# TheRealShamsaba/KnightVision

Hardware: AMD Instinct MI355X
Metric: MCTS simulations/sec + self-play games/hour (higher is better)
Workload: dtype fp32

## Files before the change

### include/kv.h

```cpp
#ifndef KV_H
#define KV_H

#include <stddef.h>
#include <stdint.h>

#ifdef __cplusplus
extern "C" {
#endif

#define KV_OK 0
#define KV_EINVAL -1
#define KV_ENOMEM -2
#define KV_EHIP -3
#define KV_EOVERFLOW -4

const char* kv_last_error(void);
int kv_version(void);

typedef struct kv_net kv_net;

size_t kv_net_packed_size(void);
int kv_net_create(int device, kv_net** out);
int kv_net_load(kv_net* net, const float* packed, size_t n_floats);
int kv_net_forward(kv_net* net, const float* planes_dev, int B, float* policy_dev, float* value_dev, void* stream);
// ... 152 lines not shown
} kv_search_result;
int kv_search(kv_engine* e, const int8_t* states , int n,
              const kv_search_params* p, kv_search_result* out );
size_t kv_sizeof_search_result(void);

int kv_search_advance(kv_engine* e, int n, const int32_t* edge , int8_t* states_out );
int kv_search_continue(kv_engine* e, int n, const kv_search_params* p, kv_search_result* out ,
                       int32_t* kept );
int kv_search_tree_size(kv_engine* e, int i, int32_t* nodes, int32_t* edges);


int kv_dev_valid_moves(int device, const int8_t* states, int n, uint16_t* moves_out, int cap, int* n_moves,
                       int8_t* states_after, uint8_t* in_check);
int kv_dev_attacks(int device, const int8_t* states, int n, uint64_t* attacked);
int kv_dev_make_move(int device, int8_t* states, const int* index, int n);
int kv_dev_dirichlet(int device, const uint64_t* seeds, int n, double alpha, int k, int draws, double* out,
                     int64_t* attempts, double* tail);
int kv_host_libm(int op, const double* x, const double* y, int n, double* out);
int kv_dev_py_random(int device, const uint64_t* seeds, int n, int count, double* out);
int kv_dev_wino88i(int device, const double* V, int rows, const double* U, int K, int digits, int seg, double* M,
                   int8_t* v_digits, int* v_exp);
int kv_dev_wino88i32_out(int device, const float* M, int rows, const float* scale, const float* shift,
                         const float* resid, int fused, float* Y, int8_t* v_digits, int* v_exp);
int kv_dev_wino88r_out(int device, const double* M, int rows, const float* scale, const float* shift,
                       const float* resid, int fused, float* Y, int8_t* v_digits, int* v_exp);
int kv_dev_i8gemm_bench(int device, int rows, int K, int variant, int iters, float* avg_us, float* M_out);
int kv_dev_gemm_clock(int device, int rows, int digits, double seconds, double* out);
int kv_dev_out_phases(int device, int rows, int resid, int r3, unsigned long long* stamps, float* us);

#define KV_PGN_OUTCOME_NONE (-128)
typedef struct kv_pgn_record {
    char fen[100];
    char san[12];
    int32_t outcome;
    int32_t game;
} kv_pgn_record;
int kv_pgn_extract(const char* text, size_t len, kv_pgn_record* out, size_t cap, size_t* n_out, size_t* consumed,
                   int64_t* n_games);
int kv_fen_codes(const char* fens, size_t stride, int n, int8_t* codes);
int kv_san_move_index(const char* fens, size_t fen_stride, const char* sans, size_t san_stride, int n,
                      int32_t* out);
int kv_chess_perft(const char* fen, int depth, uint64_t* nodes);
int kv_chess_san(const char* fen, const char* san_in, char* san_out, size_t san_cap, char* fen_after, size_t fen_cap);
int kv_chess_fen(const char* fen_in, char* fen_out, size_t cap);

int kv_tr_conv3x3_f16(const void* x_dev, int n, int ci, const void* w_dev, const float* bias_dev, int co,
// ... 38 lines not shown
```

### knightvision_amd/_lib.py

```python
from __future__ import annotations

import ctypes as C
import os

HERE = os.path.dirname(os.path.abspath(__file__))
LIB_PATH = os.environ.get("KV_LIB_PATH") or os.path.join(HERE, "libkv.so")

_lib = None


class KVError(RuntimeError):
    pass


class Config(C.Structure):
    _fields_ = [("device", C.c_int), ("slots", C.c_int), ("n_games", C.c_int64), ("game_id_base", C.c_int64),
                ("game_id_stride", C.c_int64), ("seed", C.c_uint64), ("seed_mode", C.c_int),
                ("max_moves", C.c_int), ("batch", C.c_int), ("eps", C.c_double), ("alpha", C.c_double),
                ("sims", C.c_int), ("c_puct", C.c_float), ("eval_mode", C.c_int), ("record_cap", C.c_int64),
                ("recycle", C.c_int), ("precision", C.c_int), ("algo", C.c_int), ("tree_edge_cap", C.c_int),
                ("keep_root_visits", C.c_int), ("reuse_tree", C.c_int)]


class Record(C.Structure):
# ... 97 lines not shown
        "kv_root_moves": ([vp, P(C.c_uint16), sz, P(sz)], i),
        "kv_root_moves_device": ([vp, vp, sz, P(sz), vp], i),
        "kv_records_device": ([vp, vp, sz, P(sz), vp], i),
        "kv_sync": ([vp], i),
        "kv_reset_records": ([vp], i),
        "kv_destroy": ([vp], None),
        "kv_search": ([vp, P(C.c_int8), i, P(SearchParams), P(SearchResult)], i),
        "kv_sizeof_search_result": ([], sz),
        "kv_search_advance": ([vp, i, P(C.c_int32), P(C.c_int8)], i),
        "kv_search_continue": ([vp, i, P(SearchParams), P(SearchResult), P(C.c_int32)], i),
        "kv_search_tree_size": ([vp, i, P(C.c_int32), P(C.c_int32)], i),
        "kv_dev_valid_moves": ([i, P(C.c_int8), i, P(C.c_uint16), i, P(i), P(C.c_int8), P(C.c_uint8)], i),
        "kv_dev_make_move": ([i, P(C.c_int8), P(i), i], i),
        "kv_dev_attacks": ([i, P(C.c_int8), i, P(C.c_uint64)], i),
        "kv_dev_dirichlet": ([i, P(C.c_uint64), i, C.c_double, i, i, P(C.c_double), P(i64), P(C.c_double)], i),
        "kv_dev_py_random": ([i, P(C.c_uint64), i, i, P(C.c_double)], i),
        "kv_host_libm": ([i, P(C.c_double), P(C.c_double), i, P(C.c_double)], i),
        "kv_dev_wino88i": ([i, P(C.c_double), i, P(C.c_double), i, i, i, P(C.c_double), P(C.c_int8), P(i)], i),
        "kv_dev_i8gemm_bench": ([i, i, i, i, i, P(C.c_float), P(C.c_float)], i),
        "kv_dev_gemm_clock": ([i, i, i, C.c_double, P(C.c_double)], i),
        "kv_dev_out_phases": ([i, i, i, i, P(C.c_uint64), P(C.c_float)], i),
        "kv_dev_wino88i32_out": ([i, P(C.c_float), i, P(C.c_float), P(C.c_float), P(C.c_float), i, P(C.c_float),
                                  P(C.c_int8), P(i)], i),
        "kv_dev_wino88r_out": ([i, P(C.c_double), i, P(C.c_float), P(C.c_float), P(C.c_float), i, P(C.c_float),
                                P(C.c_int8), P(i)], i),
        "kv_pgn_extract": ([C.c_char_p, sz, P(PgnRecord), sz, P(sz), P(sz), P(i64)], i),
        "kv_fen_codes": ([C.c_char_p, sz, i, P(C.c_int8)], i),
        "kv_san_move_index": ([C.c_char_p, sz, C.c_char_p, sz, i, P(C.c_int32)], i),
        "kv_chess_perft": ([C.c_char_p, i, P(C.c_uint64)], i),
        "kv_chess_san": ([C.c_char_p, C.c_char_p, C.c_char_p, sz, C.c_char_p, sz], i),
        "kv_chess_fen": ([C.c_char_p, C.c_char_p, sz], i),
        "kv_tr_conv3x3_f16": ([vp, i, i, vp, vp, i, vp, vp], i),
        "kv_tr_conv3x3_add_f16": ([vp, i, i, vp, vp, i, vp, vp, vp], i),
        "kv_tr_conv_weights_f16": ([vp, i, i, i, vp, vp, vp], i),
        "kv_tr_wgrad_workspace": ([i, i, i, P(i)], sz),
        "kv_tr_conv3x3_wgrad_f16": ([vp, vp, i, i, i, i, vp, vp, sz, vp], i),
        "kv_tr_bn_workspace": ([i, i], sz),
        "kv_tr_bn_stats_f16": ([vp, i, i, C.c_float, vp, vp, vp, vp, sz, vp], i),
        "kv_tr_bn_apply_f16": ([vp, i, i, vp, vp, vp, vp, vp, i, vp, vp], i),
        "kv_tr_bn_backward_f16": ([vp, vp, vp, i, i, i, vp, vp, vp, vp, vp, vp, vp, vp, vp, sz, vp], i),
        "kv_tr_channel_sum_f16": ([vp, i, i, vp, vp, sz, vp], i),
        "kv_tr_planes_to_nhwc": ([vp, i, i, vp, vp], i),
        "kv_tr_head1x1_f16": ([vp, i, vp, vp, vp, vp], i),
        "kv_tr_head1x1_workspace": ([i], sz),
        "kv_tr_head1x1_backward_f16": ([vp, vp, i, vp, vp, vp, vp, vp, sz, vp], i),
        "kv_tr_policy_loss_f16": ([vp, vp, vp, vp, vp, i, vp, vp, vp, vp], i),
        "kv_tr_policy_loss_backward_f16": ([vp, vp, vp, vp, vp, i, vp, vp, vp, vp, vp, vp], i),
    }
    for name, (args, res) in sig.items():
        if not hasattr(L, name):
            continue
        f = getattr(L, name)
        f.argtypes = args
        f.restype = res
    return L


EXPORTED = ["kv_last_error", "kv_version", "kv_net_packed_size", "kv_net_create", "kv_net_load", "kv_net_forward",
            "kv_net_forward_boards", "kv_net_forward_boards_legal", "kv_net_set_timing", "kv_net_last_timing", "kv_net_destroy", "kv_net_set_precision", "kv_net_set_algo",
            "kv_net_calibration", "kv_engine_calibration",
            "kv_create",
            "kv_load_weights", "kv_run", "kv_set_max_moves", "kv_records", "kv_games", "kv_stats_get", "kv_sizeof_config", "kv_sizeof_stats", "kv_root_visits", "kv_root_visits_device", "kv_root_moves", "kv_root_moves_device", "kv_records_device", "kv_sync", "kv_reset_records", "kv_destroy",
            "kv_search", "kv_sizeof_search_result", "kv_search_advance", "kv_search_continue", "kv_search_tree_size",
            "kv_dev_valid_moves", "kv_dev_make_move", "kv_dev_attacks", "kv_dev_dirichlet", "kv_dev_py_random", "kv_host_libm",
            "kv_dev_wino88i", "kv_dev_wino88i32_out", "kv_dev_wino88r_out", "kv_dev_i8gemm_bench",
            "kv_dev_gemm_clock", "kv_dev_out_phases",
            "kv_pgn_extract", "kv_fen_codes", "kv_san_move_index", "kv_chess_perft", "kv_chess_san", "kv_chess_fen",
            "kv_tr_conv3x3_f16", "kv_tr_conv3x3_add_f16", "kv_tr_conv_weights_f16", "kv_tr_wgrad_workspace", "kv_tr_conv3x3_wgrad_f16",
            "kv_tr_bn_workspace", "kv_tr_bn_stats_f16", "kv_tr_bn_apply_f16", "kv_tr_bn_backward_f16",
            "kv_tr_channel_sum_f16", "kv_tr_planes_to_nhwc", "kv_tr_head1x1_f16", "kv_tr_head1x1_workspace",
            "kv_tr_head1x1_backward_f16", "kv_tr_policy_loss_f16", "kv_tr_policy_loss_backward_f16"]


def lib():
    global _lib
    if _lib is None:
        import torch
        if not os.path.exists(LIB_PATH):
            raise KVError(f"{LIB_PATH} is missing: run `python -c 'import __graft_entry__ as g; g.build()'` "
                          "(the HIP library is required; there is no CPU fallback)")
        L = _declare(C.CDLL(LIB_PATH))
        if hasattr(L, "kv_sizeof_search_result"):
            assert L.kv_sizeof_search_result() == C.sizeof(SearchResult), "kv_search_result: ctypes mirror differs"
        if hasattr(L, "kv_sizeof_config"):
            assert L.kv_sizeof_config() == C.sizeof(Config), "kv_config: ctypes mirror differs"
            assert L.kv_sizeof_stats() == C.sizeof(Stats), "kv_stats: ctypes mirror differs"
        _lib = L
    return _lib
# ... 7 lines not shown
```

### knightvision_amd/csrc/kv_nn.hip

```cpp
#include <hip/hip_runtime.h>
#include <math.h>
#include <stdarg.h>
#include <stdlib.h>
#include <string.h>

#include <algorithm>
#include <chrono>
#include <mutex>
#include <set>
#include <utility>
#include <vector>

#include "kv_common.h"
#include "kv_wino.h"
#include "kv_wino88.h"
#include "kv_wino88d.h"
#include "kv_wino88i.h"
#include "kv_ref64.h"

namespace kv {

static thread_local char g_err[512];

void set_error(const char* fmt, ...) {
// ... 215 lines not shown
                                                           float* out) {
    const size_t i = (size_t)blockIdx.x * blockDim.x + threadIdx.x;
    if (i >= n4) return;
    const f32x4* sl = (const f32x4*)slab + i;
    f32x4 v = sl[0];
    for (int s0 = 1; s0 < splits; s0 += kReduceBatch) {
        f32x4 p[kReduceBatch];
#pragma unroll
        for (int k = 0; k < kReduceBatch; ++k)
            if (s0 + k < splits) p[k] = sl[(size_t)(s0 + k) * n4];
#pragma unroll
        for (int k = 0; k < kReduceBatch; ++k)
            if (s0 + k < splits) v += p[k];
    }
    const int c = (int)((i * 4) % (size_t)cout);
    const f32x4 sc = *(const f32x4*)(scale + c), sh = *(const f32x4*)(shift + c);
    f32x4 o = v * sc + sh;
    if (resid) o += ((const f32x4*)resid)[i];
#pragma unroll
    for (int e = 0; e < 4; ++e) o[e] = o[e] > 0.f ? o[e] : 0.f;
    ((f32x4*)out)[i] = o;
}

__global__ __launch_bounds__(1024) void heads_kernel(const float* __restrict__ X, const float* __restrict__ hw,
                                                     const float* __restrict__ hs, const float* __restrict__ hb,
                                                     const float* __restrict__ v1wT, const float* __restrict__ v1b,
                                                     const float* __restrict__ v2w, const float* __restrict__ v2b,
                                                     float* __restrict__ pfeat, float* __restrict__ value) {
    __shared__ float s_pf[128];
    __shared__ float s_v[64];
    __shared__ float s_h[512];
    __shared__ float s_red[8];
    const int b = blockIdx.x, t = threadIdx.x;
    const int p = t >> 4, q = t & 15;
    const float* xp = X + ((size_t)b * 64 + p) * 512;
    float a0 = 0.f, a1 = 0.f, a2 = 0.f;
#pragma unroll
    for (int j = 0; j < 8; ++j) {
        const int c = q * 4 + 64 * j;
        const f32x4 x = *(const f32x4*)(xp + c);
        const f32x4 w0 = *(const f32x4*)(hw + c);
        const f32x4 w1 = *(const f32x4*)(hw + 512 + c);
        const f32x4 w2 = *(const f32x4*)(hw + 1024 + c);
#pragma unroll
        for (int e = 0; e < 4; ++e) {
            a0 += x[e] * w0[e];
            a1 += x[e] * w1[e];
            a2 += x[e] * w2[e];
        }
    }
#pragma unroll
    for (int m = 1; m < 16; m <<= 1) {
        a0 += __shfl_xor(a0, m);
        a1 += __shfl_xor(a1, m);
        a2 += __shfl_xor(a2, m);
    }
    if (q == 0) {
        const float p0 = a0 * hs[0] + hb[0], p1 = a1 * hs[1] + hb[1], v = a2 * hs[2] + hb[2];
        s_pf[p] = p0 > 0.f ? p0 : 0.f;
        s_pf[64 + p] = p1 > 0.f ? p1 : 0.f;
        s_v[p] = v > 0.f ? v : 0.f;
    }
    __syncthreads();
    if (t < 128) pfeat[(size_t)b * 128 + t] = s_pf[t];
    if (t < 512) {
        float hsum = v1b[t];
#pragma unroll 16
        for (int k = 0; k < 64; ++k) hsum += v1wT[k * 512 + t] * s_v[k];
        s_h[t] = hsum > 0.f ? hsum : 0.f;
    }
    __syncthreads();
    if (t < 256) {
        float part = v2w[t] * s_h[t] + v2w[t + 256] * s_h[t + 256];
#pragma unroll
        for (int m = 32; m >= 1; m >>= 1) part += __shfl_xor(part, m);
        if ((t & 63) == 0) s_red[t >> 6] = part;
    }
    __syncthreads();
    if (t == 0) value[b] = tanhf(s_red[0] + s_red[1] + s_red[2] + s_red[3] + v2b[0]);
}

__global__ __launch_bounds__(256) void policy_fc_kernel(const float* __restrict__ pfeat,
                                                        const float* __restrict__ w, const float* __restrict__ bias,
                                                        float* __restrict__ logits, int nb) {
    const int lane = threadIdx.x & 63, wave = threadIdx.x >> 6;
    const int h = lane >> 5, li = lane & 31;
    const int n0 = blockIdx.x * 128 + wave * 32;
    const int b0 = blockIdx.y * 32;
    const int arow = min(b0 + li, nb - 1);
    const float* ap = pfeat + (size_t)arow * 128 + 4 * h;
    const float* bp = w + (size_t)(n0 + li) * 128 + 4 * h;
    f32x16 acc;
#pragma unroll
    for (int r = 0; r < 16; ++r) acc[r] = 0.f;
    f32x4 a[16], v[16];
#pragma unroll
    for (int s = 0; s < 16; ++s) {
        a[s] = *(const f32x4*)(ap + 8 * s);
        v[s] = *(const f32x4*)(bp + 8 * s);
    }
#pragma unroll
    for (int s = 0; s < 16; ++s)
// ... 343 lines not shown
static int net_reserve(kv_net* net, int nb_pad) {
    KV_REQUIRE(nb_pad <= kMaxBoards, KV_EINVAL, "kv_net: %d boards per forward (at most %d)", nb_pad, kMaxBoards);
    if (nb_pad <= net->cap) return KV_OK;
    int cap = nb_pad < 64 ? 64 : nb_pad;
    (void)hipFree(net->x16); (void)hipFree(net->X); (void)hipFree(net->T); (void)hipFree(net->pfeat);
    (void)hipFree(net->ev8); (void)hipFree(net->evmax8);
    net->x16 = net->X = net->T = net->pfeat = nullptr;
    net->ev8 = nullptr;
    net->evmax8 = nullptr;
    net->cap = 0;
    KV_HIP(hipMalloc(&net->x16, (size_t)cap * 64 * 16 * 4));
    KV_HIP(hipMalloc(&net->X, (size_t)cap * 64 * 512 * 4));
    KV_HIP(hipMalloc(&net->T, (size_t)cap * 64 * 512 * 4));
    KV_HIP(hipMalloc(&net->pfeat, (size_t)cap * 128 * 4));
    KV_HIP(hipMalloc(&net->ev8, (size_t)cap * kv::W88_XI * 2 * sizeof(int)));
    KV_HIP(hipMalloc(&net->evmax8, (size_t)cap * kv::W88_XI * sizeof(unsigned)));
    if (!net->slab)
        KV_HIP(hipMalloc(&net->slab, (size_t)(144 / kSplitKt) * kSplitMaxBoards * 64 * 512 * 4));
    net->cap = cap;
    return KV_OK;
}

static int net_heads(kv_net* net, int nb, float* policy, float* value, hipStream_t st);

template <int K, int WR, int WC, int MT, int NT, int CK, int LDS_PAD, int XI>
static int launch_wino_gemm_t(const float* V, const float* U, float* M, int rows, int stride, hipStream_t st,
                              int xi0 = 0, int nxi = XI) {
    using T = kv::WinoTile<WR, WC, MT, NT, CK>;
    constexpr size_t bytes = T::BYTES + LDS_PAD;
    KV_HIP(lds_opt_in((const void*)kv::wino_gemm_kernel<K, WR, WC, MT, NT, CK, XI>, (int)bytes));
    const int nwg = nxi * (rows / T::WM) * (512 / T::WN);
    KV_REQUIRE(rows % T::WM == 0 && nwg % 8 == 0 && xi0 >= 0 && nxi > 0 && xi0 + nxi <= XI, KV_EINVAL,
               "wino gemm: rows %d vs tile %d, points [%d, %d)", rows, T::WM, xi0, xi0 + nxi);
    hipLaunchKernelGGL((kv::wino_gemm_kernel<K, WR, WC, MT, NT, CK, XI>), dim3(nwg), dim3(T::THREADS), bytes, st, V,
                       U, M, rows, 512, stride, xi0);
    KV_HIP(hipGetLastError());
    return KV_OK;
}

static bool debug_skip_transforms() {
    static const int v = [] {
        const char* e = getenv("KV_DEBUG_SKIP_TRANSFORMS");
        return e && e[0] == '1' ? 1 : 0;
    }();
    return v != 0;
}
// ... 534 lines not shown
                                                                      kv::W88_XI, net->V8, net->ev8, st)))
            return rc;
    } else if (slice && v64) {
        KV_REQUIRE(K == 256, KV_EINVAL, "wino88i32v: the output kernels write the digits of K 512");
        if ((rc = launch_wino88i_slice<256, D>((const double*)net->V256, rows, stride, kv::W88_XI, net->V8, net->ev8,
                                               st)))
            return rc;
    } else if (slice) {
        const float* Vsrc = K == 256 ? (const float*)net->V256 : (const float*)net->V;
        rc = K == 256 ? launch_wino88i_slice<256, D>(Vsrc, rows, stride, kv::W88_XI, net->V8, net->ev8, st)
             : seg    ? launch_wino88i_slice<512, D, float, 2>(Vsrc, rows, stride, kv::W88_XI, net->V8, net->ev8, st)
                      : launch_wino88i_slice<512, D>(Vsrc, rows, stride, kv::W88_XI, net->V8, net->ev8, st);
        if (rc) return rc;
    }
    const int8_t* U = (r3 ? net->U88r3 : net->U88i32) + net->uoff88[l] * D;
    const int* eu = (r3 ? net->eu88r3 : net->eu88i32) + net->euoff[l];
    rc = K == 256 ? i8f32_gemm<256>(net->V8, net->ev8, U, eu, M, rows, stride, false, st, r3)
                  : i8f32_gemm<512>(net->V8, net->ev8, U, eu, M, rows, stride, seg, st, r3);
    if (rc) return rc;
    if (mark && net->res_b) KV_HIP(hipEventRecord(net->res_b, st));
    return KV_OK;
}

static int wino88i32_blocks(kv_net* net, int nb, bool mark, bool v64, hipStream_t st, bool r3 = false) {
    const int rows = nb, stride = rows;
    float* V = (float*)net->V;
    const float* M = (const float*)net->Mw;
    const bool sf = i8f32_form().slice && !v64 && !r3, seg = i8f32_form().seg && !v64 && !r3;
    int8_t* V8 = net->V8;
    int* ev = net->ev8;
    int rc;
    if ((rc = wino88i32_gemm_layer(net, 1, 256, rows, stride, true, false, v64, st, r3))) return rc;
    rc = v64  ? launch_wino88i32v_out<false, true>(net, 1, M, nb, stride, nullptr, net->X, V8, ev, st)
         : sf ? launch_wino88_out<false, true, true>(net, 1, M, nb, stride, nullptr, net->X, V, st)
              : launch_wino88i32_out<false, true>(net, 1, M, nb, stride, nullptr, net->X, V8, ev, seg, st, r3);
    if (rc) return rc;
    if (mark && net->timing) KV_HIP(hipEventRecord(net->ev[1], st));
    for (int r = 0; r < 5; ++r) {
        const int l1 = 2 + 2 * r, l2 = 3 + 2 * r;
        const bool m = mark && r == 2;
        if ((rc = wino88i32_gemm_layer(net, l1, 512, rows, stride, sf, m, v64, st, r3))) return rc;
        rc = v64  ? launch_wino88i32v_out<false, false>(net, l1, M, nb, stride, nullptr, nullptr, V8, ev, st)
             : sf ? launch_wino88_out<false, false, true>(net, l1, M, nb, stride, nullptr, nullptr, V, st)
                  : launch_wino88i32_out<false, false>(net, l1, M, nb, stride, nullptr, nullptr, V8, ev, seg, st, r3);
        if (rc) return rc;
        if ((rc = wino88i32_gemm_layer(net, l2, 512, rows, stride, sf, false, v64, st, r3))) return rc;
        if (r == 4)
            rc = launch_wino88_out<true, true, false>(net, l2, M, nb, stride, net->X, net->X, nullptr, st);
        else
            rc = v64  ? launch_wino88i32v_out<true, true>(net, l2, M, nb, stride, net->X, net->X, V8, ev, st)
                 : sf ? launch_wino88_out<true, true, true>(net, l2, M, nb, stride, net->X, net->X, V, st)
                      : launch_wino88i32_out<true, true>(net, l2, M, nb, stride, net->X, net->X, V8, ev, seg, st, r3);
        if (rc) return rc;
    }
    if (mark && net->timing) KV_HIP(hipEventRecord(net->ev[2], st));
    return KV_OK;
}

struct WsNeed {
    size_t b[4];
};
static WsNeed ws_need(int path) {
    constexpr size_t f = 4, d = 8, P88 = kv::W88_XI;
    switch (path) {
        case KV_PATH_WINO88: return {{P88 * 512 * f, P88 * 512 * f, P88 * 256 * f, 0}};
        case KV_PATH_WINO88_F64: return {{P88 * 512 * d, P88 * 512 * d, P88 * 256 * d, 0}};
        case KV_PATH_WINO88_I8: return {{0, P88 * 512 * d, P88 * 256 * d, P88 * 512 * kv::kI8Digits}};
        case KV_PATH_WINO88_I8R: return {{0, P88 * 512 * d, P88 * 256 * d, P88 * 512 * 4}};
        case KV_PATH_WINO88_I8F32:
            return {{i8f32_form().slice ? P88 * 512 * f : 0, P88 * 512 * f, P88 * 256 * f,
                     P88 * 512 * kv::kI8DigitsF32}};
        case KV_PATH_WINO88_I8F32V: return {{0, P88 * 512 * f, P88 * 256 * d, P88 * 512 * kv::kI8DigitsF32}};
        case KV_PATH_WINO88_I8F32R3: return {{0, P88 * 512 * f, P88 * 256 * f, P88 * 512 * kv::kI8DigitsF32}};
        default: return {{0, 0, 0, 0}};
    }
}

static int net_reserve_ws(kv_net* net, int path) {
    void** buf[4] = {&net->V, &net->Mw, &net->V256, (void**)&net->V8};
    const WsNeed n = ws_need(path);
    for (int i = 0; i < 4; ++i) {
        const size_t need = n.b[i] * (size_t)net->cap;
        if (need <= net->ws_cap[i]) continue;
        (void)hipFree(*buf[i]);
        *buf[i] = nullptr;
        net->ws_cap[i] = 0;
        KV_HIP(hipMalloc(buf[i], need));
        net->ws_cap[i] = need;
    }
    return KV_OK;
}

static int net_tower_wino(kv_net* net, int nb_pad, int path, bool v256_ready, hipStream_t st) {
    int rc;
    net->dom_path = path;
    net->dom_launches = 1;
    t_dom_kernel = nullptr;
    if (path == KV_PATH_WINO88 || path == KV_PATH_WINO88_F64 || path == KV_PATH_WINO88_I8 ||
        path == KV_PATH_WINO88_I8R || path == KV_PATH_WINO88_I8F32 || path == KV_PATH_WINO88_I8F32V ||
        path == KV_PATH_WINO88_I8F32R3) {
        const bool f64 = path == KV_PATH_WINO88_F64 || path == KV_PATH_WINO88_I8 || path == KV_PATH_WINO88_I8R ||
                         path == KV_PATH_WINO88_I8F32V;
        if (!v256_ready) {
            if (f64)
                hipLaunchKernelGGL(kv::wino88d_in_kernel<256>, dim3(1, nb_pad), dim3(256), 0, st, net->T, nb_pad,
                                   (double*)net->V256);
            else
                hipLaunchKernelGGL(kv::wino88_in_kernel<256>, dim3(1, nb_pad), dim3(256), 0, st, net->T, nb_pad,
                                   (float*)net->V256);
            KV_HIP(hipGetLastError());
        }
        if ((rc = path == KV_PATH_WINO88_I8F32    ? wino88i32_blocks(net, nb_pad, true, false, st)
                  : path == KV_PATH_WINO88_I8F32R3 ? wino88i32_blocks(net, nb_pad, true, false, st, true)
                  : path == KV_PATH_WINO88_I8F32V ? wino88i32_blocks(net, nb_pad, true, true, st)
                  : path == KV_PATH_WINO88_I8  ? wino88i_blocks(net, nb_pad, true, false, st)
                  : path == KV_PATH_WINO88_I8R ? wino88i_blocks(net, nb_pad, true, true, st)
                  : path == KV_PATH_WINO88_F64 ? wino88d_blocks(net, nb_pad, true, st)
                                               : wino88_blocks(net, nb_pad, true, st)))
            return rc;
        net->dom_flop = 2.0 * kv::W88_XI * nb_pad * 512.0 * 512.0;
        net->dom_kernel = t_dom_kernel ? t_dom_kernel : "?";
        net->dom_algo = KV_ALGO_WINOGRAD88;
        net->dom_split = path != KV_PATH_WINO88 ? 0 : (nb_pad % 128 == 0 ? wino88_split_points(nb_pad) : kv::W88_XI);
        return KV_OK;
    }
    KV_REQUIRE(false, KV_EINVAL, "kv_net: conv path %d is not a Winograd tower", path);
}

static int net_tower(kv_net* net, int nb, int nb_pad, const int8_t* boards, float* policy, float* value,
                     hipStream_t st) {
    const float* W = net->w;
    const kv::PackOffsets& o = net->off;
    int rc;
    const bool tm = net->timing;
    const int path = path_for(net, nb);
    KV_REQUIRE(net->built[path], KV_EINVAL, "kv_net: conv path %d has no weights (load the net after choosing it)",
               path);
    KV_REQUIRE(nb_pad <= net->cap, KV_EINVAL, "kv_net: %d boards over the reserved %d", nb_pad, net->cap);
    if ((rc = net_reserve_ws(net, path))) return rc;
    if (tm) KV_HIP(hipEventRecord(net->ev[0], st));
    bool v256_ready = false;
    if (boards) {
        if (path == KV_PATH_WINO88 || path == KV_PATH_WINO88_I8F32 || path == KV_PATH_WINO88_I8F32R3)
            hipLaunchKernelGGL(kv::stem_kernel<4>, dim3(4, nb_pad / 2), dim3(256), 0, st, boards, nb, net->stemT,
                               W + o.scale[0], W + o.shift[0], (float*)net->V256, nb_pad, nullptr);
        else if (path == KV_PATH_WINO88_F64 || path == KV_PATH_WINO88_I8 || path == KV_PATH_WINO88_I8R ||
                 path == KV_PATH_WINO88_I8F32V)
            hipLaunchKernelGGL(kv::stem_kernel<5>, dim3(4, nb_pad / 2), dim3(256), 0, st, boards, nb, net->stemT,
                               W + o.scale[0], W + o.shift[0], (float*)net->V256, nb_pad, nullptr);
        else
            hipLaunchKernelGGL(kv::stem_kernel<0>, dim3(4, nb_pad / 2), dim3(256), 0, st, boards, nb, net->stemT,
                               W + o.scale[0], W + o.shift[0], net->T, nb_pad * 4, nullptr);
        KV_HIP(hipGetLastError());
        v256_ready = path != KV_PATH_DIRECT;
    } else if ((rc = launch_conv<16, 16, false>(net->x16, W + o.w[0], W + o.scale[0], W + o.shift[0], nullptr,
                                                net->T, 256, nb_pad, nullptr, st))) {
        return rc;
    }
    if (path_is_wino(path)) {
        if ((rc = net_tower_wino(net, nb_pad, path, v256_ready, st))) return rc;
        return net_heads(net, nb, policy, value, st);
    }
    if ((rc = launch_conv<256, 32, false>(net->T, W + o.w[1], W + o.scale[1], W + o.shift[1], nullptr, net->X, 512,
                                          nb_pad, net->slab, st)))
        return rc;
    if (tm) KV_HIP(hipEventRecord(net->ev[1], st));
    if (net->res_a) KV_HIP(hipEventRecord(net->res_a, st));
    for (int r = 0; r < 5; ++r) {
        const int l1 = 2 + 2 * r, l2 = 3 + 2 * r;
        if ((rc = launch_conv<512, 32, false>(net->X, W + o.w[l1], W + o.scale[l1], W + o.shift[l1], nullptr, net->T,
                                              512, nb_pad, net->slab, st)))
            return rc;
        if ((rc = launch_conv<512, 32, true>(net->T, W + o.w[l2], W + o.scale[l2], W + o.shift[l2], net->X, net->X,
                                             512, nb_pad, net->slab, st)))
            return rc;
    }
    if (tm) KV_HIP(hipEventRecord(net->ev[2], st));
    if (net->res_b) KV_HIP(hipEventRecord(net->res_b, st));
    net->dom_algo = KV_ALGO_DIRECT;
    net->dom_path = KV_PATH_DIRECT;
    net->dom_split = 0;
    net->dom_kernel = "conv3x3_kernel<512,32>";
    net->dom_launches = 10;
    net->dom_flop = (double)nb_pad * 64 * 512 * 4608 * 2;
    return net_heads(net, nb, policy, value, st);
}

static int net_heads(kv_net* net, int nb, float* policy, float* value, hipStream_t st) {
    const float* W = net->w;
    const kv::PackOffsets& o = net->off;
    hipLaunchKernelGGL(kv::heads_kernel, dim3(nb), dim3(1024), 0, st, net->X, W + o.head_w, W + o.head_scale,
                       W + o.head_shift, net->v1wT, W + o.vfc1_b, W + o.vfc2_w, W + o.vfc2_b, net->pfeat, value);
    KV_HIP(hipGetLastError());
    if (net->legal.out) {
        hipLaunchKernelGGL(kv::policy_legal_kernel, dim3(nb), dim3(64), 0, st, net->pfeat, W + o.pfc_w, W + o.pfc_b,
                           net->legal.moves, net->legal.n, net->legal.maxm, net->legal.out);
    } else {
        hipLaunchKernelGGL(kv::policy_fc_kernel, dim3(4096 / 128, (nb + 31) / 32), dim3(256), 0, st, net->pfeat,
                           W + o.pfc_w, W + o.pfc_b, policy, nb);
    }
    KV_HIP(hipGetLastError());
    return KV_OK;
}

static size_t wino_offsets(size_t* uoff, int nxi) {
    size_t tot = 0;
    for (int l = 1; l < 12; ++l) {
        uoff[l] = tot;
        tot += (size_t)nxi * kv::kConv[l].cout * kv::kConv[l].cin;
    }
    return tot;
}

static int ensure_path(kv_net* net, int path) {
    if (net->built[path]) return KV_OK;
    if (path == KV_PATH_WINO88_I8F32V) {
// ... 611 lines not shown
        }
        KV_HIP(hipGetLastError());
    } else {
        if (resid)
            hipLaunchKernelGGL((kv::wino88_out_kernel<true, true, true>), dim3(512 / 256, rows), dim3(256), 0, 0,
                               dm.p, rows, sc, sh, dy.p, dy.p, dv.p);
        else
            hipLaunchKernelGGL((kv::wino88_out_kernel<false, true, true>), dim3(512 / 256, rows), dim3(256), 0, 0,
                               dm.p, rows, sc, sh, nullptr, dy.p, dv.p);
        KV_HIP(hipGetLastError());
        int rc = seg  ? launch_wino88i_slice<512, kv::kI8DigitsF32, float, 2>(dv.p, rows, rows, kv::W88_XI, v8.p, ev.p, 0)
                 : r3 ? launch_wino88i_slice<512, kv::kI8DigitsF32, float, 1, false, true>(dv.p, rows, rows, kv::W88_XI,
                                                                                           v8.p, ev.p, 0)
                      : launch_wino88i_slice<512, kv::kI8DigitsF32>(dv.p, rows, rows, kv::W88_XI, v8.p, ev.p, 0);
        if (rc) return rc;
    }
    KV_HIP(hipDeviceSynchronize());
    KV_HIP(hipMemcpy(Y, dy.p, ny * sizeof(float), hipMemcpyDeviceToHost));
    KV_HIP(hipMemcpy(v_digits, v8.p, nm * kv::kI8DigitsF32, hipMemcpyDeviceToHost));
    KV_HIP(hipMemcpy(v_exp, ev.p, (size_t)kv::W88_XI * rows * (seg ? 2 : 1) * sizeof(int), hipMemcpyDeviceToHost));
    return KV_OK;
}

int kv_dev_wino88r_out(int device, const double* M, int rows, const float* scale, const float* shift,
                       const float* resid, int fused, float* Y, int8_t* v_digits, int* v_exp) {
    KV_REQUIRE(M && scale && shift && Y && v_digits && v_exp && rows > 0 && rows % 128 == 0 && rows <= kMaxBoards,
               KV_EINVAL, "kv_dev_wino88r_out: bad arguments (rows %d: a multiple of 128, at most %d)", rows,
               kMaxBoards);
    KV_HIP(hipSetDevice(device));
    const size_t nm = (size_t)kv::W88_XI * rows * 512, ny = (size_t)rows * 64 * 512;
    kv::DevBuf<double> dm, dv;
    kv::DevBuf<float> dsc, dsh, dy;
    kv::DevBuf<int8_t> v8;
    kv::DevBuf<int> ev;
    KV_HIP(dm.alloc(nm));
    KV_HIP(dsc.alloc(512));
    KV_HIP(dsh.alloc(512));
    KV_HIP(dy.alloc(ny));
    KV_HIP(v8.alloc(nm * 4));
    KV_HIP(ev.alloc((size_t)kv::W88_XI * rows));
    KV_HIP(hipMemcpy(dm.p, M, nm * sizeof(double), hipMemcpyHostToDevice));
    KV_HIP(hipMemcpy(dsc.p, scale, 512 * sizeof(float), hipMemcpyHostToDevice));
    KV_HIP(hipMemcpy(dsh.p, shift, 512 * sizeof(float), hipMemcpyHostToDevice));
    if (resid)
        KV_HIP(hipMemcpy(dy.p, resid, ny * sizeof(float), hipMemcpyHostToDevice));
    else
// ... 356 lines not shown
```

### knightvision_amd/csrc/kv_wino88i.h

```cpp
#pragma once
#include <hip/hip_runtime.h>

#include "kv_common.h"
#include "kv_wino88.h"
#include "kv_wino88d.h"

namespace kv {

constexpr int kI8Digits = 5;
constexpr int kI8DigitsF32 = 4;

typedef int i8x16_t __attribute__((ext_vector_type(4)));
typedef int i32x16_t __attribute__((ext_vector_type(16)));

__device__ inline int i8_row_exponent(unsigned m) {
    if (!m) return 0;
    return (int)(m >> 20) - 1022 + ((m & 0xFE000u) == 0xFE000u ? 1 : 0);
}

__device__ inline int i8_row_exponent_f32(unsigned m) {
    if (!m) return 0;
    return (int)(m >> 23) - 126 + ((m & 0x7F0000u) == 0x7F0000u ? 1 : 0);
}

// ... 1716 lines not shown
            const int xi = a * 10 + bb;
            const unsigned P = i8f32_digits<R3>(vk[aa][bb], exs[xi]);
            {
                const unsigned T4 = i8_quad_transpose(P, lane);
                if constexpr (!R3)
                    __builtin_nontemporal_store(T4, &dst[(off0 + (unsigned)xi * xstride) >> 2]);
                else if (q < 3)
                    dst[(off0 + (unsigned)xi * xstride) >> 2] = T4;
            }
        }
    }
    if constexpr (STAMP) {
        st[4] = __builtin_amdgcn_s_memtime();
        asm volatile("s_waitcnt vmcnt(0)" ::: "memory");
        st[5] = __builtin_amdgcn_s_memtime();
        if (stamper) {
            unsigned long long* o = kOutStamps[b][w == 0 ? 0 : 1];
#pragma unroll
            for (int k = 0; k < 6; ++k) o[k] = st[k];
        }
    }
}

template <bool RESID, bool WRITE_Y, bool R3 = false>
__global__ __launch_bounds__(1024) void wino88i32_outp_kernel(const float* __restrict__ M, int rows,
                                                              const float* __restrict__ scale,
                                                              const float* __restrict__ shift, const float* resid,
                                                              float* Y, int8_t* __restrict__ V8,
                                                              int* __restrict__ ex) {
#pragma clang fp contract(off)
    constexpr int NK = 512 / 32, NW = 16, NSLOT = 3, SLOT = 20 * 2048;
    extern __shared__ __attribute__((aligned(16))) char lds_outp[];
    unsigned(*red)[2][5][16] = (unsigned(*)[2][5][16])(lds_outp + NSLOT * SLOT);
    int* exs = (int*)(lds_outp + NSLOT * SLOT + NW * 2 * 5 * 16 * 4);
    const int lane = threadIdx.x & 63, w = threadIdx.x >> 6, h = lane >> 5;
    const int wu = __builtin_amdgcn_readfirstlane(w);
    const int c = w * 32 + (lane & 31);
    const int G = (int)gridDim.x;
    const int nbw = ((int)rows - (int)blockIdx.x + G - 1) / G;
    const int nsteps = 5 * nbw;
    const int npieces = wu < 8 ? 3 : 2;
    const float sc = scale[c], sh = shift[c];
    const unsigned xs = (unsigned)rows * 512;
    auto issue = [&](int t) {
        if (t >= nsteps) return;
        const int b = (int)blockIdx.x + (t / 5) * G, jj = t % 5;
// ... 251 lines not shown
```

Before: 318,500.

## Fuse stem with int8 Winograd input and last output transform with heads

Adds a stem_r3 kernel that computes the stem convolution and writes int8 Winograd digits directly, skipping the fp32 V256 buffer and the separate slicing pass for large batches on the R3 path. Adds a fused kernel that runs the final residual Winograd output transform and the policy/value heads per board in LDS, so the last activation is not written to global memory and re-read. The heads math is switched to explicit FMAs, which may change numerics slightly. Test entry points for both fused paths are exported.

```diff
diff --git a/include/kv.h b/include/kv.h
--- a/include/kv.h
+++ b/include/kv.h
@@ -198,6 +198,10 @@
                    int8_t* v_digits, int* v_exp);
 int kv_dev_wino88i32_out(int device, const float* M, int rows, const float* scale, const float* shift,
                          const float* resid, int fused, float* Y, int8_t* v_digits, int* v_exp);
+int kv_dev_tower_front(int device, const int8_t* boards, int nb, int rows, const float* wT, const float* scale,
+                       const float* shift, int fused, int8_t* v_digits, int* v_exp);
+int kv_dev_tower_back(int device, const float* M, int rows, const float* scale, const float* shift,
+                      const float* resid, const float* heads, int fused, float* pfeat, float* value);
 int kv_dev_wino88r_out(int device, const double* M, int rows, const float* scale, const float* shift,
                        const float* resid, int fused, float* Y, int8_t* v_digits, int* v_exp);
 int kv_dev_i8gemm_bench(int device, int rows, int K, int variant, int iters, float* avg_us, float* M_out);
diff --git a/knightvision_amd/_lib.py b/knightvision_amd/_lib.py
--- a/knightvision_amd/_lib.py
+++ b/knightvision_amd/_lib.py
@@ -143,6 +143,10 @@
         "kv_dev_out_phases": ([i, i, i, i, P(C.c_uint64), P(C.c_float)], i),
         "kv_dev_wino88i32_out": ([i, P(C.c_float), i, P(C.c_float), P(C.c_float), P(C.c_float), i, P(C.c_float),
                                   P(C.c_int8), P(i)], i),
+        "kv_dev_tower_front": ([i, P(C.c_int8), i, i, P(C.c_float), P(C.c_float), P(C.c_float), i, P(C.c_int8),
+                                P(i)], i),
+        "kv_dev_tower_back": ([i, P(C.c_float), i, P(C.c_float), P(C.c_float), P(C.c_float), P(C.c_float), i,
+                               P(C.c_float), P(C.c_float)], i),
         "kv_dev_wino88r_out": ([i, P(C.c_double), i, P(C.c_float), P(C.c_float), P(C.c_float), i, P(C.c_float),
                                 P(C.c_int8), P(i)], i),
         "kv_pgn_extract": ([C.c_char_p, sz, P(PgnRecord), sz, P(sz), P(sz), P(i64)], i),
@@ -184,7 +188,7 @@
             "kv_load_weights", "kv_run", "kv_set_max_moves", "kv_records", "kv_games", "kv_stats_get", "kv_sizeof_config", "kv_sizeof_stats", "kv_root_visits", "kv_root_visits_device", "kv_root_moves", "kv_root_moves_device", "kv_records_device", "kv_sync", "kv_reset_records", "kv_destroy",
             "kv_search", "kv_sizeof_search_result", "kv_search_advance", "kv_search_continue", "kv_search_tree_size",
             "kv_dev_valid_moves", "kv_dev_make_move", "kv_dev_attacks", "kv_dev_dirichlet", "kv_dev_py_random", "kv_host_libm",
-            "kv_dev_wino88i", "kv_dev_wino88i32_out", "kv_dev_wino88r_out", "kv_dev_i8gemm_bench",
+            "kv_dev_wino88i", "kv_dev_wino88i32_out", "kv_dev_wino88r_out", "kv_dev_tower_front", "kv_dev_tower_back", "kv_dev_i8gemm_bench",
             "kv_dev_gemm_clock", "kv_dev_out_phases",
             "kv_pgn_extract", "kv_fen_codes", "kv_san_move_index", "kv_chess_perft", "kv_chess_san", "kv_chess_fen",
             "kv_tr_conv3x3_f16", "kv_tr_conv3x3_add_f16", "kv_tr_conv_weights_f16", "kv_tr_wgrad_workspace", "kv_tr_conv3x3_wgrad_f16",
diff --git a/knightvision_amd/csrc/kv_nn.hip b/knightvision_amd/csrc/kv_nn.hip
--- a/knightvision_amd/csrc/kv_nn.hip
+++ b/knightvision_amd/csrc/kv_nn.hip
@@ -261,18 +261,19 @@
     ((f32x4*)out)[i] = o;
 }
 
-__global__ __launch_bounds__(1024) void heads_kernel(const float* __restrict__ X, const float* __restrict__ hw,
-                                                     const float* __restrict__ hs, const float* __restrict__ hb,
-                                                     const float* __restrict__ v1wT, const float* __restrict__ v1b,
-                                                     const float* __restrict__ v2w, const float* __restrict__ v2b,
-                                                     float* __restrict__ pfeat, float* __restrict__ value) {
+__device__ inline void heads_board(const float* xb, int b, const float* __restrict__ hw,
+                                   const float* __restrict__ hs, const float* __restrict__ hb,
+                                   const float* __restrict__ v1wT, const float* __restrict__ v1b,
+                                   const float* __restrict__ v2w, const float* __restrict__ v2b,
+                                   float* __restrict__ pfeat, float* __restrict__ value) {
+#pragma clang fp contract(off)
     __shared__ float s_pf[128];
     __shared__ float s_v[64];
     __shared__ float s_h[512];
     __shared__ float s_red[8];
-    const int b = blockIdx.x, t = threadIdx.x;
+    const int t = threadIdx.x;
     const int p = t >> 4, q = t & 15;
-    const float* xp = X + ((size_t)b * 64 + p) * 512;
+    const float* xp = xb + (size_t)p * 512;
     float a0 = 0.f, a1 = 0.f, a2 = 0.f;
 #pragma unroll
     for (int j = 0; j < 8; ++j) {
@@ -283,9 +284,9 @@
         const f32x4 w2 = *(const f32x4*)(hw + 1024 + c);
 #pragma unroll
         for (int e = 0; e < 4; ++e) {
-            a0 += x[e] * w0[e];
-            a1 += x[e] * w1[e];
-            a2 += x[e] * w2[e];
+            a0 = __builtin_fmaf(x[e], w0[e], a0);
+            a1 = __builtin_fmaf(x[e], w1[e], a1);
+            a2 = __builtin_fmaf(x[e], w2[e], a2);
         }
     }
 #pragma unroll
@@ -295,7 +296,8 @@
         a2 += __shfl_xor(a2, m);
     }
     if (q == 0) {
-        const float p0 = a0 * hs[0] + hb[0], p1 = a1 * hs[1] + hb[1], v = a2 * hs[2] + hb[2];
+        const float p0 = __builtin_fmaf(a0, hs[0], hb[0]), p1 = __builtin_fmaf(a1, hs[1], hb[1]),
+                    v = __builtin_fmaf(a2, hs[2], hb[2]);
         s_pf[p] = p0 > 0.f ? p0 : 0.f;
         s_pf[64 + p] = p1 > 0.f ? p1 : 0.f;
         s_v[p] = v > 0.f ? v : 0.f;
@@ -305,18 +307,50 @@
     if (t < 512) {
         float hsum = v1b[t];
 #pragma unroll 16
-        for (int k = 0; k < 64; ++k) hsum += v1wT[k * 512 + t] * s_v[k];
+        for (int k = 0; k < 64; ++k) hsum = __builtin_fmaf(v1wT[k * 512 + t], s_v[k], hsum);
         s_h[t] = hsum > 0.f ? hsum : 0.f;
     }
     __syncthreads();
     if (t < 256) {
-        float part = v2w[t] * s_h[t] + v2w[t + 256] * s_h[t + 256];
+        float part = __builtin_fmaf(v2w[t], s_h[t], v2w[t + 256] * s_h[t + 256]);
 #pragma unroll
         for (int m = 32; m >= 1; m >>= 1) part += __shfl_xor(part, m);
         if ((t & 63) == 0) s_red[t >> 6] = part;
     }
     __syncthreads();
     if (t == 0) value[b] = tanhf(s_red[0] + s_red[1] + s_red[2] + s_red[3] + v2b[0]);
+}
+
+__global__ __launch_bounds__(1024) void heads_kernel(const float* __restrict__ X, const float* __restrict__ hw,
+                                                     const float* __restrict__ hs, const float* __restrict__ hb,
+                                                     const float* __restrict__ v1wT, const float* __restrict__ v1b,
+                                                     const float* __restrict__ v2w, const float* __restrict__ v2b,
+                                                     float* __restrict__ pfeat, float* __restrict__ value) {
+    const int b = blockIdx.x;
+    heads_board(X + (size_t)b * 64 * 512, b, hw, hs, hb, v1wT, v1b, v2w, v2b, pfeat, value);
+}
+
+constexpr int kOutHeadsLds = 64 * 512 * 4;
+template <bool YNT>
+__global__ __launch_bounds__(1024) void wino88_out_heads_kernel(
+    const float* __restrict__ M, int rows, const float* __restrict__ scale, const float* __restrict__ shift,
+    const float* __restrict__ resid, const float* __restrict__ hw, const float* __restrict__ hs,
+    const float* __restrict__ hb, const float* __restrict__ v1wT, const float* __restrict__ v1b,
+    const float* __restrict__ v2w, const float* __restrict__ v2b, float* __restrict__ pfeat,
+    float* __restrict__ value) {
+    extern __shared__ __attribute__((aligned(16))) float xs[];
+    const int lane = threadIdx.x & 63, w = threadIdx.x >> 6, h = lane >> 5;
+    const int c = w * 32 + (lane & 31), b = blockIdx.x;
+    {
+        float x2[4][8];
+        wino88_out_plane_half<true, false, false, 0, YNT>(M, rows, b, c, h, scale[c], shift[c], resid, nullptr, x2);
+#pragma unroll
+        for (int ii = 0; ii < 4; ++ii)
+#pragma unroll
+            for (int j = 0; j < 8; ++j) xs[((4 * h + ii) * 8 + j) * 512 + c] = x2[ii][j];
+    }
+    __syncthreads();
+    heads_board(xs, b, hw, hs, hb, v1wT, v1b, v2w, v2b, pfeat, value);
 }
 
 __global__ __launch_bounds__(256) void policy_fc_kernel(const float* __restrict__ pfeat,
@@ -706,6 +740,7 @@
 }
 
 static int net_heads(kv_net* net, int nb, float* policy, float* value, hipStream_t st);
+static int net_policy(kv_net* net, int nb, float* policy, hipStream_t st);
 
 template <int K, int WR, int WC, int MT, int NT, int CK, int LDS_PAD, int XI>
 static int launch_wino_gemm_t(const float* V, const float* U, float* M, int rows, int stride, hipStream_t st,
@@ -1286,7 +1321,38 @@
     return KV_OK;
 }
 
-static int wino88i32_blocks(kv_net* net, int nb, bool mark, bool v64, hipStream_t st, bool r3 = false) {
+static int launch_wino88_out_heads(const float* M, int nb, int stride, const float* sc, const float* sh,
+                                   const float* resid, const float* hw, const float* hs, const float* hb,
+                                   const float* v1wT, const float* v1b, const float* v2w, const float* v2b,
+                                   float* pfeat, float* value, bool ynt, hipStream_t st) {
+    auto kern = ynt ? kv::wino88_out_heads_kernel<true> : kv::wino88_out_heads_kernel<false>;
+    KV_HIP(lds_opt_in((const void*)kern, kv::kOutHeadsLds));
+    hipLaunchKernelGGL(kern, dim3(nb), dim3(1024), kv::kOutHeadsLds, st, M, stride, sc, sh, resid, hw, hs, hb, v1wT,
+                       v1b, v2w, v2b, pfeat, value);
+    KV_HIP(hipGetLastError());
+    return KV_OK;
+}
+
+static int launch_stem_r3(const int8_t* boards, int nb, int rows, const float* stemT, const float* sc,
+                          const float* sh, int8_t* V8, int* ev, hipStream_t st) {
+    KV_REQUIRE(rows % 32 == 0 && nb <= rows, KV_EINVAL, "R3 stem: %d boards in %d rows (a multiple of 32: out_board)",
+               nb, rows);
+    const int cus = device_cus() & ~7;
+    const int grid = cus > 0 && cus < rows ? cus : rows;
+    KV_HIP(lds_opt_in((const void*)kv::stem_r3_kernel, kv::kStemR3Lds));
+    hipLaunchKernelGGL(kv::stem_r3_kernel, dim3(grid), dim3(512), kv::kStemR3Lds, st, boards, nb, rows, stemT, sc, sh,
+                       V8, ev);
+    KV_HIP(hipGetLastError());
+    return KV_OK;
+}
+
+struct HeadsOut {
+    int nb;
+    float* value;
+};
+
+static int wino88i32_blocks(kv_net* net, int nb, bool mark, bool v64, hipStream_t st, bool r3 = false,
+                            const HeadsOut* ho = nullptr, bool v8_ready = false) {
     const int rows = nb, stride = rows;
     float* V = (float*)net->V;
     const float* M = (const float*)net->Mw;
@@ -1294,7 +1360,7 @@
     int8_t* V8 = net->V8;
     int* ev = net->ev8;
     int rc;
-    if ((rc = wino88i32_gemm_layer(net, 1, 256, rows, stride, true, false, v64, st, r3))) return rc;
+    if ((rc = wino88i32_gemm_layer(net, 1, 256, rows, stride, !v8_ready, false, v64, st, r3))) return rc;
     rc = v64  ? launch_wino88i32v_out<false, true>(net, 1, M, nb, stride, nullptr, net->X, V8, ev, st)
          : sf ? launch_wino88_out<false, true, true>(net, 1, M, nb, stride, nullptr, net->X, V, st)
               : launch_wino88i32_out<false, true>(net, 1, M, nb, stride, nullptr, net->X, V8, ev, seg, st, r3);
@@ -1309,7 +1375,13 @@
                   : launch_wino88i32_out<false, false>(net, l1, M, nb, stride, nullptr, nullptr, V8, ev, seg, st, r3);
         if (rc) return rc;
         if ((rc = wino88i32_gemm_layer(net, l2, 512, rows, stride, sf, false, v64, st, r3))) return rc;
-        if (r == 4)
+        if (r == 4 && ho) {
+            const float* W = net->w;
+            const kv::PackOffsets& o = net->off;
+            rc = launch_wino88_out_heads(M, ho->nb, stride, W + o.scale[l2], W + o.shift[l2], net->X, W + o.head_w,
+                                         W + o.head_scale, W + o.head_shift, net->v1wT, W + o.vfc1_b, W + o.vfc2_w,
+                                         W + o.vfc2_b, net->pfeat, ho->value, ho->nb >= 1024, st);
+        } else if (r == 4)
             rc = launch_wino88_out<true, true, false>(net, l2, M, nb, stride, net->X, net->X, nullptr, st);
         else
             rc = v64  ? launch_wino88i32v_out<true, true>(net, l2, M, nb, stride, net->X, net->X, V8, ev, st)
@@ -1355,7 +1427,8 @@
     return KV_OK;
 }
 
-static int net_tower_wino(kv_net* net, int nb_pad, int path, bool v256_ready, hipStream_t st) {
+static int net_tower_wino(kv_net* net, int nb_pad, int path, bool v256_ready, hipStream_t st,
+                          const HeadsOut* ho = nullptr, bool v8_ready = false) {
     int rc;
     net->dom_path = path;
     net->dom_launches = 1;
@@ -1365,7 +1438,7 @@
         path == KV_PATH_WINO88_I8F32R3) {
         const bool f64 = path == KV_PATH_WINO88_F64 || path == KV_PATH_WINO88_I8 || path == KV_PATH_WINO88_I8R ||
                          path == KV_PATH_WINO88_I8F32V;
-        if (!v256_ready) {
+        if (!v256_ready && !v8_ready) {
             if (f64)
                 hipLaunchKernelGGL(kv::wino88d_in_kernel<256>, dim3(1, nb_pad), dim3(256), 0, st, net->T, nb_pad,
                                    (double*)net->V256);
@@ -1374,9 +1447,9 @@
                                    (float*)net->V256);
             KV_HIP(hipGetLastError());
         }
-        if ((rc = path == KV_PATH_WINO88_I8F32    ? wino88i32_blocks(net, nb_pad, true, false, st)
-                  : path == KV_PATH_WINO88_I8F32R3 ? wino88i32_blocks(net, nb_pad, true, false, st, true)
-                  : path == KV_PATH_WINO88_I8F32V ? wino88i32_blocks(net, nb_pad, true, true, st)
+        if ((rc = path == KV_PATH_WINO88_I8F32    ? wino88i32_blocks(net, nb_pad, true, false, st, false, ho)
+                  : path == KV_PATH_WINO88_I8F32R3 ? wino88i32_blocks(net, nb_pad, true, false, st, true, ho, v8_ready)
+                  : path == KV_PATH_WINO88_I8F32V ? wino88i32_blocks(net, nb_pad, true, true, st, false, ho)
                   : path == KV_PATH_WINO88_I8  ? wino88i_blocks(net, nb_pad, true, false, st)
                   : path == KV_PATH_WINO88_I8R ? wino88i_blocks(net, nb_pad, true, true, st)
                   : path == KV_PATH_WINO88_F64 ? wino88d_blocks(net, nb_pad, true, st)
@@ -1403,8 +1476,13 @@
     KV_REQUIRE(nb_pad <= net->cap, KV_EINVAL, "kv_net: %d boards over the reserved %d", nb_pad, net->cap);
     if ((rc = net_reserve_ws(net, path))) return rc;
     if (tm) KV_HIP(hipEventRecord(net->ev[0], st));
-    bool v256_ready = false;
-    if (boards) {
+    bool v256_ready = false, v8_ready = false;
+    if (boards && path == KV_PATH_WINO88_I8F32R3 && nb_pad >= 1024) {
+        if ((rc = launch_stem_r3(boards, nb, nb_pad, net->stemT, W + o.scale[0], W + o.shift[0], net->V8, net->ev8,
+                                 st)))
+            return rc;
+        v8_ready = true;
+    } else if (boards) {
         if (path == KV_PATH_WINO88 || path == KV_PATH_WINO88_I8F32 || path == KV_PATH_WINO88_I8F32R3)
             hipLaunchKernelGGL(kv::stem_kernel<4>, dim3(4, nb_pad / 2), dim3(256), 0, st, boards, nb, net->stemT,
                                W + o.scale[0], W + o.shift[0], (float*)net->V256, nb_pad, nullptr);
@@ -1422,6 +1500,11 @@
         return rc;
     }
     if (path_is_wino(path)) {
+        if (path == KV_PATH_WINO88_I8F32 || path == KV_PATH_WINO88_I8F32R3 || path == KV_PATH_WINO88_I8F32V) {
+            const HeadsOut ho = {nb, value};
+            if ((rc = net_tower_wino(net, nb_pad, path, v256_ready, st, &ho, v8_ready))) return rc;
+            return net_policy(net, nb, policy, st);
+        }
         if ((rc = net_tower_wino(net, nb_pad, path, v256_ready, st))) return rc;
         return net_heads(net, nb, policy, value, st);
     }
@@ -1456,6 +1539,12 @@
     hipLaunchKernelGGL(kv::heads_kernel, dim3(nb), dim3(1024), 0, st, net->X, W + o.head_w, W + o.head_scale,
                        W + o.head_shift, net->v1wT, W + o.vfc1_b, W + o.vfc2_w, W + o.vfc2_b, net->pfeat, value);
     KV_HIP(hipGetLastError());
+    return net_policy(net, nb, policy, st);
+}
+
+static int net_policy(kv_net* net, int nb, float* policy, hipStream_t st) {
+    const float* W = net->w;
+    const kv::PackOffsets& o = net->off;
     if (net->legal.out) {
         hipLaunchKernelGGL(kv::policy_legal_kernel, dim3(nb), dim3(64), 0, st, net->pfeat, W + o.pfc_w, W + o.pfc_b,
                            net->legal.moves, net->legal.n, net->legal.maxm, net->legal.out);
@@ -2113,6 +2202,91 @@
     return KV_OK;
 }
 
+int kv_dev_tower_front(int device, const int8_t* boards, int nb, int rows, const float* wT, const float* scale,
+                       const float* shift, int fused, int8_t* v_digits, int* v_exp) {
+    KV_REQUIRE(boards && wT && scale && shift && v_digits && v_exp && nb > 0 && nb <= rows && rows % 32 == 0 &&
+                   rows <= kMaxBoards,
+               KV_EINVAL, "kv_dev_tower_front: bad arguments (%d boards in %d rows: a multiple of 32, at most %d)", nb,
+               rows, kMaxBoards);
+    KV_HIP(hipSetDevice(device));
+    const size_t nv = (size_t)kv::W88_XI * rows * 256, nd = nv * kv::kI8DigitsF32;
+    kv::DevBuf<int8_t> db, v8;
+    kv::DevBuf<float> dw, dsc, dsh, dv;
+    kv::DevBuf<int> ev;
+    KV_HIP(db.alloc((size_t)nb * 64));
+    KV_HIP(dw.alloc(9 * 12 * 256));
+    KV_HIP(dsc.alloc(256));
+    KV_HIP(dsh.alloc(256));
+    KV_HIP(v8.alloc(nd));
+    KV_HIP(ev.alloc((size_t)kv::W88_XI * rows));
+    KV_HIP(hipMemset(v8.p, 0x55, nd));
+    KV_HIP(hipMemcpy(db.p, boards, (size_t)nb * 64, hipMemcpyHostToDevice));
+    KV_HIP(hipMemcpy(dw.p, wT, 9 * 12 * 256 * sizeof(float), hipMemcpyHostToDevice));
+    KV_HIP(hipMemcpy(dsc.p, scale, 256 * sizeof(float), hipMemcpyHostToDevice));
+    KV_HIP(hipMemcpy(dsh.p, shift, 256 * sizeof(float), hipMemcpyHostToDevice));
+    if (fused) {
+        const int rc = launch_stem_r3(db.p, nb, rows, dw.p, dsc.p, dsh.p, v8.p, ev.p, 0);
+        if (rc) return rc;
+    } else {
+        KV_HIP(dv.alloc(nv));
+        hipLaunchKernelGGL(kv::stem_kernel<4>, dim3(4, rows / 2), dim3(256), 0, 0, db.p, nb, dw.p, dsc.p, dsh.p, dv.p,
+                           rows, nullptr);
+        KV_HIP(hipGetLastError());
+        const int rc = launch_wino88i_slice<256, kv::kI8DigitsF32, float, 1, false, true>(dv.p, rows, rows, kv::W88_XI,
+                                                                                          v8.p, ev.p, 0);
+        if (rc) return rc;
+    }
+    KV_HIP(hipDeviceSynchronize());
+    KV_HIP(hipMemcpy(v_digits, v8.p, nd, hipMemcpyDeviceToHost));
+    KV_HIP(hipMemcpy(v_exp, ev.p, (size_t)kv::W88_XI * rows * sizeof(int), hipMemcpyDeviceToHost));
+    return KV_OK;
+}
+
+int kv_dev_tower_back(int device, const float* M, int rows, const float* scale, const float* shift,
+                      const float* resid, const float* heads, int fused, float* pfeat, float* value) {
+    KV_REQUIRE(M && scale && shift && resid && heads && pfeat && value && rows > 0 && rows % 32 == 0 &&
+                   rows <= kMaxBoards,
+               KV_EINVAL, "kv_dev_tower_back: bad arguments (rows %d: a multiple of 32, at most %d)", rows,
+               kMaxBoards);
+    KV_HIP(hipSetDevice(device));
+    const size_t nm = (size_t)kv::W88_XI * rows * 512, ny = (size_t)rows * 64 * 512;
+    constexpr size_t kHeads = 3 * 512 + 3 + 3 + 512 * 64 + 512 + 512 + 1;
+    kv::DevBuf<float> dm, dsc, dsh, dy, dh, dwT, dpf, dval;
+    KV_HIP(dm.alloc(nm));
+    KV_HIP(dsc.alloc(512));
+    KV_HIP(dsh.alloc(512));
+    KV_HIP(dy.alloc(ny));
+    KV_HIP(dh.alloc(kHeads));
+    KV_HIP(dwT.alloc(64 * 512));
+    KV_HIP(dpf.alloc((size_t)rows * 128));
+    KV_HIP(dval.alloc(rows));
+    KV_HIP(hipMemcpy(dm.p, M, nm * sizeof(float), hipMemcpyHostToDevice));
+    KV_HIP(hipMemcpy(dsc.p, scale, 512 * sizeof(float), hipMemcpyHostToDevice));
+    KV_HIP(hipMemcpy(dsh.p, shift, 512 * sizeof(float), hipMemcpyHostToDevice));
+    KV_HIP(hipMemcpy(dy.p, resid, ny * sizeof(float), hipMemcpyHostToDevice));
+    KV_HIP(hipMemcpy(dh.p, heads, kHeads * sizeof(float), hipMemcpyHostToDevice));
+    const float *hw = dh.p, *hs = hw + 3 * 512, *hb = hs + 3, *v1w = hb + 3, *v1b = v1w + 512 * 64,
+                *v2w = v1b + 512, *v2b = v2w + 512;
+    hipLaunchKernelGGL(kv::transpose_v1_kernel, dim3(64 * 512 / 256), dim3(256), 0, 0, v1w, dwT.p);
+    KV_HIP(hipGetLastError());
+    if (fused) {
+        const int rc = launch_wino88_out_heads(dm.p, rows, rows, dsc.p, dsh.p, dy.p, hw, hs, hb, dwT.p, v1b, v2w, v2b,
+                                               dpf.p, dval.p, (fused & 2) != 0, 0);
+        if (rc) return rc;
+    } else {
+        hipLaunchKernelGGL((kv::wino88_out_kernel<true, true, false>), dim3(512 / 256, rows), dim3(256), 0, 0, dm.p,
+                           rows, dsc.p, dsh.p, dy.p, dy.p, nullptr);
+        KV_HIP(hipGetLastError());
+        hipLaunchKernelGGL(kv::heads_kernel, dim3(rows), dim3(1024), 0, 0, dy.p, hw, hs, hb, dwT.p, v1b, v2w, v2b,
+                           dpf.p, dval.p);
+        KV_HIP(hipGetLastError());
+    }
+    KV_HIP(hipDeviceSynchronize());
+    KV_HIP(hipMemcpy(pfeat, dpf.p, (size_t)rows * 128 * sizeof(float), hipMemcpyDeviceToHost));
+    KV_HIP(hipMemcpy(value, dval.p, (size_t)rows * sizeof(float), hipMemcpyDeviceToHost));
+    return KV_OK;
+}
+
 int kv_dev_wino88r_out(int device, const double* M, int rows, const float* scale, const float* shift,
                        const float* resid, int fused, float* Y, int8_t* v_digits, int* v_exp) {
     KV_REQUIRE(M && scale && shift && Y && v_digits && v_exp && rows > 0 && rows % 128 == 0 && rows <= kMaxBoards,
diff --git a/knightvision_amd/csrc/kv_wino88i.h b/knightvision_amd/csrc/kv_wino88i.h
--- a/knightvision_amd/csrc/kv_wino88i.h
+++ b/knightvision_amd/csrc/kv_wino88i.h
@@ -1762,6 +1762,96 @@
     }
 }
 
+constexpr int kStemR3Lds = 9 * 13 * 256 * 4;
+__global__ __launch_bounds__(512) void stem_r3_kernel(const int8_t* __restrict__ boards, int nb, int rows,
+                                                      const float* __restrict__ wT, const float* __restrict__ scale,
+                                                      const float* __restrict__ shift, int8_t* __restrict__ V8,
+                                                      int* __restrict__ ex) {
+#pragma clang fp contract(off)
+    constexpr int NK = 256 / 32, NW = 8;
+    extern __shared__ __attribute__((aligned(16))) float stem_wl[];
+    __shared__ int codes[100];
+    __shared__ __attribute__((aligned(16))) unsigned red[NW][2][5][16];
+    __shared__ int exs[100];
+    const int lane = threadIdx.x & 63, w = threadIdx.x >> 6, h = lane >> 5;
+    const int c = w * 32 + (lane & 31);
+    for (int i = threadIdx.x; i < 9 * 13 * 256; i += 512) {
+        const int r = i >> 8, code = r / 9, t = r % 9;
+        stem_wl[i] = code ? wT[(size_t)(t * 12 + code - 1) * 256 + (i & 255)] : 0.f;
+    }
+    const float sc = scale[c], sh = shift[c];
+    const int q = lane & 3;
+    unsigned* const dst = (unsigned*)V8;
+    const unsigned xstride = NK * (unsigned)rows * 96u;
+    for (int id = blockIdx.x; id < rows; id += gridDim.x) {
+        const int b = out_board<true>(id);
+        __syncthreads();
+        if (threadIdx.x < 100) {
+            const int i = threadIdx.x, r = i / 10 - 1, f = i % 10 - 1;
+            const bool in = b < nb && r >= 0 && r < 8 && f >= 0 && f < 8;
+            codes[i] = in ? boards[(size_t)b * 64 + r * 8 + f] * (9 * 256) : 0;
+        }
+        __syncthreads();
+        float vk[5][10];
+        {
+            float t2[10][4];
+            {
+                float x2[4][8];
+#pragma unroll
+                for (int ii = 0; ii < 4; ++ii)
+#pragma unroll
+                    for (int px = 0; px < 8; ++px) {
+                        const int py = 4 * h + ii;
+                        float acc = 0.f;
+#pragma unroll
+                        for (int t = 0; t < 9; ++t)
+                            acc += stem_wl[codes[(py + t / 3) * 10 + px + t % 3] + t * 256 + c];
+                        const float v = __builtin_fmaf(acc, sc, sh);
+                        x2[ii][px] = v > 0.f ? v : 0.f;
+                    }
+                wino88_input_cols(x2, h, t2);
+            }
+#pragma unroll
+            for (int aa = 0; aa < 5; ++aa) wino88_input_row(t2, h, aa, vk[aa]);
+        }
+#pragma unroll
+        for (int aa = 0; aa < 5; ++aa) {
+            unsigned m[10];
+#pragma unroll
+            for (int bb = 0; bb < 10; ++bb) m[bb] = i8_half_max_dpp(__float_as_uint(vk[aa][bb]) & 0x7fffffffu);
+            if ((lane & 31) == 16) {
+                uint4* rr = (uint4*)&red[w][h][aa][0];
+                rr[0] = make_uint4(m[0], m[1], m[2], m[3]);
+                rr[1] = make_uint4(m[4], m[5], m[6], m[7]);
+                *(uint2*)&red[w][h][aa][8] = make_uint2(m[8], m[9]);
+            }
+        }
+        __syncthreads();
+        if (threadIdx.x < 100) {
+            const int xi = threadIdx.x, a = xi / 10, bb = xi % 10, hh = a / 5, aa = a % 5;
+            unsigned m = 0;
+#pragma unroll
+            for (int ww = 0; ww < NW; ++ww) m = red[ww][hh][aa][bb] > m ? red[ww][hh][aa][bb] : m;
+            const int e = i8_row_exponent_f32r(m);
+            exs[xi] = e;
+            ex[(size_t)xi * rows + b] = e;
+        }
+        __syncthreads();
+        const unsigned off0 = ((unsigned)(c >> 5) * rows + b) * 96u + q * 32 + (c & 28);
+#pragma unroll
+        for (int aa = 0; aa < 5; ++aa) {
+            const int a = 5 * h + aa;
+#pragma unroll
+            for (int bb = 0; bb < 10; ++bb) {
+                const int xi = a * 10 + bb;
+                const unsigned P = i8_digits_r3((double)vk[aa][bb], exs[xi]);
+                const unsigned T4 = i8_quad_transpose(P, lane);
+                if (q < 3) dst[(off0 + (unsigned)xi * xstride) >> 2] = T4;
+            }
+        }
+    }
+}
+
 template <bool RESID, bool WRITE_Y, bool R3 = false>
 __global__ __launch_bounds__(1024) void wino88i32_outp_kernel(const float* __restrict__ M, int rows,
                                                               const float* __restrict__ scale,
```

Measured after the change: 324,900, median of 6. 2.0% higher.
